# DIAGNijmegen/bodyct-dram-emph-subtype

Hardware: AMD Instinct MI355X
Metric: CT volumes/sec (train step, 1x128x256x256) (higher is better)
Workload: dtype f32; 1 GPU; BASELINE configs[1]: resnet18segcls train step (fwd+loss+bwd+Adam), batch 2/GPU, 1x128x256x256, fp32, inputs resident in HBM; global_batch=2, parallelism=dp1, hip_graph=False, streams=2

## Files before the change

### bodyct-dram-emph-subtype_amd/csrc/stem.hip

```cpp
#include "common.h"

namespace {

constexpr int PZ = 13, PY = 21, PX = 21;
constexpr int PATCH = PZ * PY * PX;
constexpr int PXP = 24;
constexpr int PATCHP = PZ * PY * PXP;
constexpr int WLP = 96;
constexpr int KT = 50;
constexpr int WPT = (KT * 64 + 255) / 256;

struct StemGeom {
  int B, D, H, W, Do, Ho, Wo;
  int nz, ny, nx, tiles_per_b, nblk;
};

template <typename T>
__global__ __launch_bounds__(256, 2) void stem_fwd_kernel(const float* __restrict__ x,
                                                          const float* __restrict__ w,
                                                          T* __restrict__ y, float* __restrict__ stats,
                                                          const StemGeom g) {
  __shared__ __attribute__((aligned(16))) float lds[PATCHP + KT * WLP];
  float* patch = lds;
  float* wl = lds + PATCHP;
  const int tid = threadIdx.x, lane = tid & 63, wave = tid >> 6;
  const int li = lane & 31, lh = lane >> 5;

  int L = xcd_remap(blockIdx.x, g.nblk);
  const int b = L / g.tiles_per_b;
  int r = L - b * g.tiles_per_b;
  const int txi = r % g.nx; r /= g.nx;
  const int tyi = r % g.ny;
  const int tzi = r / g.ny;
  const int z0 = tzi * 4, y0 = tyi * 8, x0 = txi * 8;

  for (int idx = tid; idx < PATCH; idx += 256) {
    const int pz = idx / (PY * PX);
    const int rem = idx - pz * (PY * PX);
    const int py = rem / PX, px = rem - py * PX;
    const int zi = 2 * z0 - 3 + pz, yi = 2 * y0 - 3 + py, xi = 2 * x0 - 3 + px;
    const bool ok = (zi >= 0) & (zi < g.D) & (yi >= 0) & (yi < g.H) & (xi >= 0) & (xi < g.W);
    patch[(pz * PY + py) * PXP + px] = ok ? x[(((long)b * g.D + zi) * g.H + yi) * g.W + xi] : 0.f;
  }

  float rw[WPT];
  auto load_w = [&](int kz) {
#pragma unroll
    for (int p = 0; p < WPT; ++p) {
      const int idx = p * 256 + tid;
      const int t = idx >> 6, co = idx & 63;
      rw[p] = (idx < KT * 64 && t < 49) ? w[co * 343 + kz * 49 + t] : 0.f;
    }
  };
  auto store_w = [&]() {
#pragma unroll
    for (int p = 0; p < WPT; ++p) {
      const int idx = p * 256 + tid;
      if (idx < KT * 64) wl[(idx >> 6) * WLP + (idx & 63)] = rw[p];
    }
  };

  f32x16 acc[2][2];
#pragma unroll
  for (int mi = 0; mi < 2; ++mi)
#pragma unroll
    for (int nj = 0; nj < 2; ++nj)
#pragma unroll
      for (int e = 0; e < 16; ++e) acc[mi][nj][e] = 0.f;

  int abase[2];
#pragma unroll
  for (int mi = 0; mi < 2; ++mi) abase[mi] = (2 * wave) * (PY * PXP) + (2 * (4 * mi + (li >> 3))) * PXP + 2 * (li & 7);

  load_w(0);
  for (int kz = 0; kz < 7; ++kz) {
    __syncthreads();
    store_w();
    __syncthreads();
    if (kz + 1 < 7) load_w(kz + 1);
    const float* pk = patch + kz * (PY * PXP);
#pragma unroll
    for (int kk = 0; kk < KT / 2; ++kk) {
      constexpr int dummy = 0;
      (void)dummy;
      const int k0 = 2 * kk, k1 = 2 * kk + 1;
      const int o0 = (k0 < 49) ? (k0 / 7) * PXP + (k0 % 7) : 0;
      const int o1 = (k1 < 49) ? (k1 / 7) * PXP + (k1 % 7) : 0;
      const int ko = lh ? o1 : o0;
      const float a0 = pk[abase[0] + ko];
      const float a1 = pk[abase[1] + ko];
      const float b0 = wl[(2 * kk + lh) * WLP + li];
      const float b1 = wl[(2 * kk + lh) * WLP + 32 + li];
      acc[0][0] = __builtin_amdgcn_mfma_f32_32x32x2f32(a0, b0, acc[0][0], 0, 0, 0);
      acc[0][1] = __builtin_amdgcn_mfma_f32_32x32x2f32(a0, b1, acc[0][1], 0, 0, 0);
      acc[1][0] = __builtin_amdgcn_mfma_f32_32x32x2f32(a1, b0, acc[1][0], 0, 0, 0);
      acc[1][1] = __builtin_amdgcn_mfma_f32_32x32x2f32(a1, b1, acc[1][1], 0, 0, 0);
    }
  }

  float s1[2] = {0.f, 0.f}, s2[2] = {0.f, 0.f};
#pragma unroll
  for (int mi = 0; mi < 2; ++mi) {
#pragma unroll
    for (int e = 0; e < 16; ++e) {
      const int row = wave * 64 + mi * 32 + (e & 3) + 8 * (e >> 2) + 4 * lh;
      const int zo = z0 + (row >> 6), yo = y0 + ((row >> 3) & 7), xo = x0 + (row & 7);
      if ((zo < g.Do) & (yo < g.Ho) & (xo < g.Wo)) {
        const long o = ((((long)b * g.Do + zo) * g.Ho + yo) * g.Wo + xo) * 64 + li;
#pragma unroll
        for (int nj = 0; nj < 2; ++nj) {
          const float v = acc[mi][nj][e];
          st1<T>(y, o + nj * 32, v);
          s1[nj] += v;
          s2[nj] += v * v;
        }
      }
    }
  }
  if (stats) {
    __syncthreads();
    float* red = lds;
#pragma unroll
    for (int nj = 0; nj < 2; ++nj) {
      const float t1 = s1[nj] + __shfl_xor(s1[nj], 32, 64);
      const float t2 = s2[nj] + __shfl_xor(s2[nj], 32, 64);
      if (lh == 0) {
        red[(wave * 2 + 0) * 64 + nj * 32 + li] = t1;
        red[(wave * 2 + 1) * 64 + nj * 32 + li] = t2;
      }
    }
    __syncthreads();
    if (tid < 128) {
      const int which = tid >> 6, c = tid & 63;
      const float v = red[(0 + which) * 64 + c] + red[(2 + which) * 64 + c] + red[(4 + which) * 64 + c] +
                      red[(6 + which) * 64 + c];
      stats[((long)L * 2 + which) * 64 + c] = v;
    }
  }
}

constexpr int GZ = 7, GY = 21, GX = 21;
constexpr int GPATCH = GZ * GY * GX;
constexpr int GXP = 27;
constexpr int GPATCHP = GZ * GY * GXP;
constexpr int NTAP = 352;
constexpr int GLDY = 96;
constexpr int GPT = (GPATCH + 255) / 256;

struct StemWGeom {
  int B, D, H, W, Do, Ho, Wo;
  int ny, nx;
  int total;
};

template <typename T>
__global__ __launch_bounds__(256, 2) void stem_wgrad_kernel(const float* __restrict__ x,
                                                            const T* __restrict__ dy,
                                                            float* __restrict__ slab, const StemWGeom g) {
  __shared__ __attribute__((aligned(16))) float lds[GPATCHP + 3 + 64 * GLDY];
  float* patch = lds;
  float* dyl = lds + GPATCHP + 3;
  const int tid = threadIdx.x, lane = tid & 63, wave = tid >> 6;
  const int li = lane & 31, lh = lane >> 5;
  const int ntw = (wave < 3) ? 3 : 2;

  int toff[3];
#pragma unroll
  for (int j = 0; j < 3; ++j) {
    const int tap = 32 * (wave + 4 * j) + li;
    const int kz = tap / 49, rem = tap - kz * 49, ky = rem / 7, kx = rem - ky * 7;
    toff[j] = (tap < 343 ? kz * (GY * GXP) + ky * GXP + kx : 0) + 2 * lh;
  }

  f32x16 acc[3][2];
#pragma unroll
  for (int j = 0; j < 3; ++j)
#pragma unroll
    for (int mi = 0; mi < 2; ++mi)
#pragma unroll
      for (int e = 0; e < 16; ++e) acc[j][mi][e] = 0.f;

  float rp[GPT];
  float4 rd[4];
  auto load_tile = [&](int st) {
    int r = st;
    const int txi = r % g.nx; r /= g.nx;
    const int tyi = r % g.ny; r /= g.ny;
    const int zo = r % g.Do;
    const int b = r / g.Do;
    const int y0 = tyi * 8, x0 = txi * 8;
#pragma unroll
    for (int p = 0; p < GPT; ++p) {
      const int idx = p * 256 + tid;
      const int pz = idx / (GY * GX);
      const int rem = idx - pz * (GY * GX);
      const int py = rem / GX, px = rem - py * GX;
      const int zi = 2 * zo - 3 + pz, yi = 2 * y0 - 3 + py, xi = 2 * x0 - 3 + px;
      const bool ok = (idx < GPATCH) & (zi >= 0) & (zi < g.D) & (yi >= 0) & (yi < g.H) & (xi >= 0) & (xi < g.W);
      rp[p] = ok ? x[(((long)b * g.D + zi) * g.H + yi) * g.W + xi] : 0.f;
    }
#pragma unroll
    for (int p = 0; p < 4; ++p) {
      const int idx = p * 256 + tid;
      const int v = idx >> 4, c4 = idx & 15;
      const int yo = y0 + (v >> 3), xo = x0 + (v & 7);
      const bool ok = (yo < g.Ho) & (xo < g.Wo);
      const long o = ((((long)b * g.Do + zo) * g.Ho + yo) * g.Wo + xo) * 64 + c4 * 4;
      rd[p] = ok ? ld4<T>(dy, o) : make_float4(0.f, 0.f, 0.f, 0.f);
    }
  };
  auto store_tile = [&]() {
#pragma unroll
    for (int p = 0; p < GPT; ++p) {
      const int idx = p * 256 + tid;
      if (idx < GPATCH) {
        const int pz = idx / (GY * GX), rem = idx - pz * (GY * GX);
        patch[(pz * GY + rem / GX) * GXP + rem % GX] = rp[p];
      }
    }
#pragma unroll
    for (int p = 0; p < 4; ++p) {
      const int idx = p * 256 + tid;
      *reinterpret_cast<float4*>(&dyl[(idx >> 4) * GLDY + (idx & 15) * 4]) = rd[p];
    }
  };

  int st = blockIdx.x;
  if (st < g.total) load_tile(st);
  for (; st < g.total; st += gridDim.x) {
    __syncthreads();
    store_tile();
    __syncthreads();
    if (st + (int)gridDim.x < g.total) load_tile(st + gridDim.x);
#pragma unroll 8
    for (int kk = 0; kk < 32; ++kk) {
      const int vbase = (2 * (kk >> 2)) * GXP + 4 * (kk & 3);
      const float a0 = dyl[(2 * kk + lh) * GLDY + li];
      const float a1 = dyl[(2 * kk + lh) * GLDY + 32 + li];
#pragma unroll
      for (int j = 0; j < 3; ++j) {
        if (j < ntw) {
          const float bv = patch[vbase + toff[j]];
          acc[j][0] = __builtin_amdgcn_mfma_f32_32x32x2f32(a0, bv, acc[j][0], 0, 0, 0);
          acc[j][1] = __builtin_amdgcn_mfma_f32_32x32x2f32(a1, bv, acc[j][1], 0, 0, 0);
        }
      }
    }
  }
  float* sl = slab + (long)blockIdx.x * 64 * NTAP;
#pragma unroll
  for (int j = 0; j < 3; ++j) {
    if (j < ntw) {
#pragma unroll
      for (int mi = 0; mi < 2; ++mi)
#pragma unroll
        for (int e = 0; e < 16; ++e) {
          const int co = 32 * mi + (e & 3) + 8 * (e >> 2) + 4 * lh;
          sl[co * NTAP + 32 * (wave + 4 * j) + li] = acc[j][mi][e];
        }
    }
  }
}

__global__ __launch_bounds__(256) void stem_wgrad_reduce_kernel(const float* __restrict__ slab, float* __restrict__ dw,
                                                                int nslab) {
  __shared__ float part[4][64];
  const int r = threadIdx.x & 63, kg = threadIdx.x >> 6;
  const int i = blockIdx.x * 64 + r;
  const bool live = i < 64 * NTAP;
  float p[8];
#pragma unroll
  for (int j = 0; j < 8; ++j) p[j] = 0.f;
  if (live) {
    int k = kg;
    for (; k + 28 < nslab; k += 32) {
#pragma unroll
      for (int j = 0; j < 8; ++j) p[j] += slab[(long)(k + 4 * j) * 64 * NTAP + i];
    }
    for (int j = 0; k < nslab; k += 4, ++j) p[j] += slab[(long)k * 64 * NTAP + i];
  }
  part[kg][r] = ((p[0] + p[1]) + (p[2] + p[3])) + ((p[4] + p[5]) + (p[6] + p[7]));
  __syncthreads();
  if (kg == 0 && live) {
    const int co = i / NTAP, tap = i - co * NTAP;
    if (tap < 343) dw[co * 343 + tap] = (part[0][r] + part[1][r]) + (part[2][r] + part[3][r]);
  }
}

inline int stem_out(int n) { return (n + 6 - 7) / 2 + 1; }
inline int stem_wgrad_blocks(int total) { return total < 512 ? total : 512; }

}

extern "C" int dram_stem_num_tiles(int B, int Do, int Ho, int Wo) {
  return B * ((Do + 3) / 4) * ((Ho + 7) / 8) * ((Wo + 7) / 8);
}

template <typename T>
static int stem_fwd_impl(const float* x, const float* w, T* y, float* stats_partial, int B, int D, int H, int W,
                         dram_stream_t stream) {
  if (!x || !w || !y || B < 1 || D < 1 || H < 1 || W < 1) return DRAM_ERR_BAD_ARG;
  StemGeom g{};
  g.B = B; g.D = D; g.H = H; g.W = W;
  g.Do = stem_out(D); g.Ho = stem_out(H); g.Wo = stem_out(W);
  if ((long long)B * g.Do * g.Ho * g.Wo * 64 >= (1LL << 31)) return DRAM_ERR_UNSUPPORTED;
  g.nz = (g.Do + 3) / 4; g.ny = (g.Ho + 7) / 8; g.nx = (g.Wo + 7) / 8;
  g.tiles_per_b = g.nz * g.ny * g.nx;
  g.nblk = B * g.tiles_per_b;
  const double vo = (double)B * g.Do * g.Ho * g.Wo;
  DramProf prof(DRAM_FAM_STEM, 0, 2.0 * vo * 64.0 * 343.0,
                4.0 * ((double)B * D * H * W + 64.0 * 343.0) + sizeof(T) * vo * 64.0, (hipStream_t)stream);
  hipLaunchKernelGGL((stem_fwd_kernel<T>), dim3(g.nblk), dim3(256), 0, (hipStream_t)stream, x, w, y, stats_partial, g);
  DRAM_LAUNCH_CHECK();
  return DRAM_OK;
}
extern "C" int dram_stem_fwd(const float* x, const float* w, float* y, float* stats_partial, int B, int D,
                             int H, int W, dram_stream_t stream) {
  return stem_fwd_impl<float>(x, w, y, stats_partial, B, D, H, W, stream);
}
extern "C" int dram_stem_fwd_bf16(const float* x, const float* w, void* y, float* stats_partial, int B, int D,
                                  int H, int W, dram_stream_t stream) {
  return stem_fwd_impl<bf16_t>(x, w, (bf16_t*)y, stats_partial, B, D, H, W, stream);
}

extern "C" size_t dram_stem_bwd_weight_workspace(int B, int D, int H, int W) {
  const int Do = stem_out(D), Ho = stem_out(H), Wo = stem_out(W);
  const int total = B * Do * ((Ho + 7) / 8) * ((Wo + 7) / 8);
  return (size_t)stem_wgrad_blocks(total) * 64 * NTAP * sizeof(float);
}

template <typename T>
static int stem_bwd_weight_impl(const float* x, const T* dy, float* dw, int B, int D, int H, int W, void* workspace,
                                size_t workspace_bytes, dram_stream_t stream) {
  if (!x || !dy || !dw || B < 1 || D < 1 || H < 1 || W < 1) return DRAM_ERR_BAD_ARG;
  StemWGeom g{};
  g.B = B; g.D = D; g.H = H; g.W = W;
  g.Do = stem_out(D); g.Ho = stem_out(H); g.Wo = stem_out(W);
  g.ny = (g.Ho + 7) / 8; g.nx = (g.Wo + 7) / 8;
  g.total = B * g.Do * g.ny * g.nx;
  const int nblk = stem_wgrad_blocks(g.total);
  if (!workspace || workspace_bytes < (size_t)nblk * 64 * NTAP * sizeof(float)) return DRAM_ERR_WORKSPACE;
  hipStream_t s = (hipStream_t)stream;
  const double vo = (double)B * g.Do * g.Ho * g.Wo;
  DramProf prof(DRAM_FAM_STEM, 1, 2.0 * vo * 64.0 * 343.0,
                4.0 * ((double)B * D * H * W + 64.0 * 343.0) + sizeof(T) * vo * 64.0, s);
  hipLaunchKernelGGL((stem_wgrad_kernel<T>), dim3(nblk), dim3(256), 0, s, x, dy, (float*)workspace, g);
  DRAM_LAUNCH_CHECK();
  hipLaunchKernelGGL(stem_wgrad_reduce_kernel, dim3((64 * NTAP + 63) / 64), dim3(256), 0, s,
                     (const float*)workspace, dw, nblk);
  DRAM_LAUNCH_CHECK();
  return DRAM_OK;
}
extern "C" int dram_stem_bwd_weight(const float* x, const float* dy, float* dw, int B, int D, int H, int W,
                                    void* workspace, size_t workspace_bytes, dram_stream_t stream) {
  return stem_bwd_weight_impl<float>(x, dy, dw, B, D, H, W, workspace, workspace_bytes, stream);
}
extern "C" int dram_stem_bwd_weight_bf16(const float* x, const void* dy, float* dw, int B, int D, int H, int W,
                                         void* workspace, size_t workspace_bytes, dram_stream_t stream) {
  return stem_bwd_weight_impl<bf16_t>(x, (const bf16_t*)dy, dw, B, D, H, W, workspace, workspace_bytes, stream);
}
```

### include/dram_hip.h

```cpp
#ifndef DRAM_HIP_H
#define DRAM_HIP_H

#include <stddef.h>
#include <stdint.h>

#ifdef __cplusplus
extern "C" {
#endif

typedef void* dram_stream_t;

#define DRAM_OK 0
#define DRAM_ERR_BAD_ARG (-1)
#define DRAM_ERR_UNSUPPORTED (-2)
#define DRAM_ERR_WORKSPACE (-3)

#define DRAM_ABI_VERSION 7
int dram_version(void);
const char* dram_build_info(void);
const char* dram_abi_hash(void);
unsigned long long dram_stream_capture_id(dram_stream_t stream);

enum {
  DRAM_FAM_CONV_WINO2D = 0,
  DRAM_FAM_WINO_IN,
  DRAM_FAM_WINO_GEMM_NN,
  DRAM_FAM_WINO_OUT,
  DRAM_FAM_WINO_GEMM_TN,
  DRAM_FAM_WINO_WGRAD_OUT,
  DRAM_FAM_WEIGHT_PACK,
  DRAM_FAM_WGRAD_W2D,
  DRAM_FAM_CONV_IGEMM,
  DRAM_FAM_CONV_WGRAD,
  DRAM_FAM_STEM,
  DRAM_FAM_BN,
  DRAM_FAM_POOL_UP,
  DRAM_FAM_HEAD_LOSS,
  DRAM_FAM_OPTIM,
  DRAM_FAM_PREP,
  DRAM_FAM_CONV_BF16,
  DRAM_FAM_WGRAD_BF16,
  DRAM_FAM_COUNT
};
typedef struct DramProfRecord {
  int32_t family;
  int32_t variant;
  double mfma_flops;
  double alg_flops;
  double hbm_bytes;
  float ms;
  float pad_;
} DramProfRecord;
const char* dram_profile_family_name(int family);
int dram_profile_family_is_mfma(int family);
int dram_profile_start(int max_records);
int dram_profile_stop(void);
int dram_profile_dropped(void);
int dram_profile_read(DramProfRecord* out, int max_records);

typedef struct DramConvDesc {
  int32_t B;
  int32_t D, H, W, Cin;
  int32_t Do, Ho, Wo, Cout;
  int32_t k;
  int32_t stride, pad, dil;
  int32_t flags;
} DramConvDesc;
#define DRAM_CONV_ROUNDING_TOLERANT 1
#define DRAM_CONV_BWD_OVERLAPPED 2

int dram_pack_conv_weight(const float* w, float* wf, float* wb, int Cout, int Cin, int taps,
                          dram_stream_t stream);

int dram_conv3d_fwd(const float* x, const float* wf, const float* bias, float* y,
                    float* stats_partial, const DramConvDesc* desc, dram_stream_t stream);

int dram_conv3d_bwd_data(const float* dy, const float* wb, float* dx, const float* add,
                         const float* gate, const DramConvDesc* desc, dram_stream_t stream);

size_t dram_conv3d_bwd_weight_workspace(const DramConvDesc* desc);
int dram_conv3d_bwd_weight(const float* x, const float* dy, float* dw, const DramConvDesc* desc,
                           void* workspace, size_t workspace_bytes, dram_stream_t stream);

int dram_conv_num_mtiles(const DramConvDesc* desc);

int dram_wino_applicable(const DramConvDesc* desc);
int dram_conv_wgrad_algo(const DramConvDesc* desc);
int dram_wino_num_points(const DramConvDesc* desc);
int dram_wino_num_points_bwd(const DramConvDesc* desc);
int dram_wino_pack_weight(const float* w, float* uf, float* ub, const DramConvDesc* desc, dram_stream_t stream);
size_t dram_wino_workspace(const DramConvDesc* desc, int pass);
int dram_wino_num_stat_rows(const DramConvDesc* desc);
size_t dram_wino_v_elems(const DramConvDesc* desc);
int dram_wino_conv3d_fwd(const float* x, const float* uf, const float* bias, float* y,
                         float* stats_partial, float* v_keep, const DramConvDesc* desc, void* workspace,
                         size_t workspace_bytes, dram_stream_t stream);
int dram_wino_prologue_supported(const DramConvDesc* d);
int dram_wino_conv3d_fwd_cat(const float* x0, int C0, const float* x1, int C1, const float* uf, const float* bias, float* y,
                             float* stats_partial, float* v_keep, const DramConvDesc* desc, void* workspace,
                             size_t workspace_bytes, dram_stream_t stream);
int dram_wino_conv3d_fwd_bn(const float* x_pre, const float* pscale, const float* pshift, const float* uf, const float* bias,
                            float* y, float* stats_partial, float* v_keep, const DramConvDesc* d, void* workspace,
                            size_t workspace_bytes, dram_stream_t stream);
int dram_wino_conv3d_bwd_data(const float* dy, const float* ub, float* dx, const float* add,
                              const float* gate, const DramConvDesc* desc, void* workspace,
                              size_t workspace_bytes, dram_stream_t stream);
int dram_wino_num_stat_rows_bwd(const DramConvDesc* desc);
int dram_wino_conv3d_bwd_data_bn(const float* dy, const float* ub, float* dx, const float* bn_y, const float* bn_mean,
                                 const float* bn_invstd, const float* bn_scale, const float* bn_shift,
                                 float* stats_partial, const DramConvDesc* desc, void* workspace, size_t workspace_bytes,
                                 dram_stream_t stream);
int dram_wino_conv3d_bwd_weight(const float* x, const float* v_cache, const float* dy, float* dw,
                                const DramConvDesc* desc, void* workspace, size_t workspace_bytes,
                                dram_stream_t stream);

int dram_wino2d_applicable(const DramConvDesc* desc);
int dram_wino2d_num_stat_rows(const DramConvDesc* desc);
int dram_wino2d_pack_weight(const float* w, float* uf, float* ub, int Cout, int Cin, dram_stream_t stream);
int dram_wino2d_conv3d_fwd(const float* x, const float* uf, const float* bias, float* y,
                           float* stats_partial, const DramConvDesc* desc, dram_stream_t stream);
int dram_wino2d_conv3d_bwd_data(const float* dy, const float* ub, float* dx, const float* add,
                                const float* gate, const DramConvDesc* desc, dram_stream_t stream);

int dram_wgrad_w2d_applicable(const DramConvDesc* desc);
size_t dram_wgrad_w2d_workspace(const DramConvDesc* desc);
int dram_wgrad_w2d(const float* x, const float* dy, float* dw, const DramConvDesc* desc, void* workspace,
                   size_t workspace_bytes, dram_stream_t stream);

int dram_conv1x1_applicable(const DramConvDesc* desc);
int dram_conv1x1_num_stat_rows(const DramConvDesc* desc);
int dram_conv1x1_fwd(const float* x, const float* w2d, const float* bias, float* y, float* stats_partial,
                     const DramConvDesc* desc, dram_stream_t stream);
int dram_conv1x1_bwd_data(const float* dy, const float* wt, float* dx, const float* add, const float* gate,
                          const DramConvDesc* desc, dram_stream_t stream);
size_t dram_conv1x1_bwd_weight_workspace(const DramConvDesc* desc);
int dram_conv1x1_bwd_weight(const float* x, const float* dy, float* dw, const DramConvDesc* desc, void* workspace,
                            size_t workspace_bytes, dram_stream_t stream);

int dram_conv_algo(const DramConvDesc* desc);

int dram_stem_num_tiles(int B, int Do, int Ho, int Wo);
int dram_stem_fwd(const float* x, const float* w, float* y, float* stats_partial, int B, int D, int H,
                  int W, dram_stream_t stream);
size_t dram_stem_bwd_weight_workspace(int B, int D, int H, int W);
int dram_stem_bwd_weight(const float* x, const float* dy, float* dw, int B, int D, int H, int W,
                         void* workspace, size_t workspace_bytes, dram_stream_t stream);
size_t dram_stem_bwd_data_workspace(int B, int D, int H, int W);
int dram_stem_bwd_data(const float* dy, const float* w, float* dx, int B, int D, int H, int W, void* workspace,
                       size_t workspace_bytes, dram_stream_t stream);

int dram_reduce_partials_stages(int nparts);
#define DRAM_FOLD_TICKET_DOUBLES 256
int dram_fold_partials_stages(int nparts);
int dram_fold_partials(const float* partial, double* sums, double* scratch, float* sums_f32, float* f32_row1, int nparts,
                       int R, int C, double tail, int has_tail, dram_stream_t stream);
int dram_bn_fold_finalize(const float* partial, double* sums, double* scratch, int nparts, int C, double count,
                          const float* gamma, const float* beta, float* running_mean, float* running_var, float momentum,
                          float eps, int update_running, float* mean, float* invstd, float* scale, float* shift,
                          dram_stream_t stream);
int dram_reduce_partials(const float* partial, double* sums, double* scratch, int nparts, int R, int C,
                         double tail, int has_tail, dram_stream_t stream);

int dram_bn_finalize(const double* sums, double count, const double* count_dev, const float* gamma, const float* beta,
                     float* running_mean, float* running_var, float momentum, float eps,
                     int update_running, float* mean, float* invstd, float* scale, float* shift,
                     int C, dram_stream_t stream);

int dram_bn_apply(const float* y, const float* scale, const float* shift, const float* residual,
                  int Dr, int Hr, int Wr, int Cr, int rs, float* z, int B, int D, int H, int W, int C,
                  int relu, dram_stream_t stream);

int dram_colsum_nparts(long long rows, int C);
int dram_bn_bwd_reduce(const float* dz, const float* z, const float* y, const float* mean,
                       const float* invstd, const float* scale, const float* shift, float* partial,
                       long long rows, int C, int relu, dram_stream_t stream);
int dram_bn_bwd_apply_nparts(long long rows, int C);
int dram_bn_bwd_apply(const float* dz, const float* z, const float* y, const float* mean,
                      const float* invstd, const float* gamma, const float* scale, const float* shift,
                      const double* sums, double count, const double* count_dev, float* dy,
                      float* colsum_partial, long long rows, int C, int relu, dram_stream_t stream);
int dram_bn_bwd_apply_eval(const float* dz, const float* z, const float* y, const float* scale, const float* shift,
                           float* dy, float* colsum_partial, long long rows, int C, int relu, dram_stream_t stream);
int dram_colsum(const float* a, float* partial, long long rows, int C, dram_stream_t stream);

int dram_maxpool_fwd(const float* x, float* y, uint8_t* argmax, int B, int D, int H, int W, int C,
                     dram_stream_t stream);
int dram_bn_maxpool_fwd(const float* y, const float* scale, const float* shift, float* z, float* pooled, uint8_t* argmax,
                        int B, int D, int H, int W, int C, dram_stream_t stream);
int dram_maxpool_bwd(const float* dy, const uint8_t* argmax, const float* add, int add_stride, float* dx,
                     int B, int D, int H, int W, int C, dram_stream_t stream);

int dram_upcat_fwd(const float* src, const float* skip, float* cat, int B, int Ds, int Hs, int Ws, int Cu,
                   int Dk, int Hk, int Wk, int Ck, dram_stream_t stream);
int dram_upcat_bwd(const float* dcat, float* dsrc, float* dskip, int B, int Ds, int Hs, int Ws, int Cu,
                   int Dk, int Hk, int Wk, int Ck, dram_stream_t stream);

int dram_upmix_stat_rows(long long nvox);
int dram_upmix_axis_fwd(const void* in, int in_bf16, float* out, long long outer, int Ni, int m, int C,
                        dram_stream_t stream);
int dram_upmix_axis_fwd_final(const float* in, const void* base, void* out, int out_bf16, float* stats, long long outer,
                              int Ni, int m, int C, dram_stream_t stream);
int dram_upmix_axis_bwd(const void* g, int g_bf16, void* h, int h_bf16, long long outer, int Ni, int m, int C,
                        dram_stream_t stream);
int dram_upmix_split_weight(const float* w, float* wlo, float* ws, int Co, int Cu, int Cs, dram_stream_t stream);
int dram_upmix_merge_wgrad(const float* dwlo, const float* dws, float* dw, int Co, int Cu, int Cs, dram_stream_t stream);

int dram_head_nblk(long long voxels_per_sample);
int dram_head_fwd(const float* x, const float* w, const float* bias, const float* lungs, int Dl, int Hl,
                  int Wl, float* dense, float* partial, int B, int D, int H, int W, int NO, int sigmoid,
                  dram_stream_t stream);
int dram_head_bwd_nparts(long long voxels_per_sample);
int dram_head_bwd(const float* x, const float* w, const float* dense, const float* gdense,
                  const float* gpool, const float* lungs, int Dl, int Hl, int Wl, float* dx,
                  float* wpartial, int B, int D, int H, int W, int NO, int sigmoid, dram_stream_t stream);

#define DRAM_CAM_GRADCAM 0
#define DRAM_CAM_HIRESCAM 1
#define DRAM_CAM_LAYERCAM 2
int dram_cam_nblk(long long voxels_per_sample);
int dram_cam_point(const float* x, const float* w, const float* bias, const float* gdense, const float* gpool,
                   const float* lungs, int Dl, int Hl, int Wl, float* out, int B, int D, int H, int W, int NO,
                   int sigmoid, int method, int relu, dram_stream_t stream);
int dram_cam_sum(const float* x, const float* w, const float* bias, const float* gdense, const float* gpool,
                 const float* lungs, int Dl, int Hl, int Wl, float* partial, int B, int D, int H, int W, int NO,
                 int sigmoid, dram_stream_t stream);
int dram_cam_combine(const float* x, const float* w, const double* sums, float* out, int B, int D, int H, int W,
                     int NO, int relu, dram_stream_t stream);

int dram_segloss_nblk(long long voxels_total);
int dram_segloss_fwd(const float* cle, const float* pse, const float* lungs, const float* ems,
                     const float* binary, int Dl, int Hl, int Wl, float* partial, int B, int D, int H,
                     int W, float smoothness, dram_stream_t stream);
int dram_segloss_bwd(const float* cle, const float* pse, const float* lungs, const float* ems,
                     const float* binary, int Dl, int Hl, int Wl, const float* coef, float* gcle,
                     float* gpse, int B, int D, int H, int W, float smoothness, dram_stream_t stream);

int dram_regloss_tail(const float* partial, int nblk, const float* reg_cle, const float* reg_pse,
                      const long long* cle_labels, const long long* pse_labels, const float* cle_w,
                      const float* pse_w, const float* cle_bands, int n_cle, const float* pse_bands, int n_pse,
                      int B, double voxels_total, double smooth, double beta, double gamma, float* out,
                      float* coef, float* greg, dram_stream_t stream);

int dram_upproject_nblk(long long voxels_per_sample);
int dram_upproject(const float* dense, const float* ess, float* out, float* partial, int B, int D, int H,
                   int W, int Do, int Ho, int Wo, dram_stream_t stream);

int dram_region_nblk(long long voxels_per_sample);
int dram_upproject_regions(const float* cle, const float* pse, long long dense_batch_stride, const uint8_t* ess,
                           const uint8_t* labels, float* out_cle, float* out_pse, float* partial, double* table, int B,
                           int D, int H, int W, int Do, int Ho, int Wo, int n_regions, dram_stream_t stream);
int dram_prep_labels(const void* labels, int label_dtype, long long stride_z, long long stride_y, const int* zidx,
                     uint8_t* out, int D, int H, int W, int Do, int Ho, int Wo, dram_stream_t stream);

#define DRAM_HEAT_CLASSSUM 0
#define DRAM_HEAT_PLAIN 1
int dram_heat_nblk(long long voxels_per_sample);
int dram_heat_peak(const float* dense, long long stride_b, long long stride_c, int C, float* partial, int B, int d,
                   int h, int w, int D, int H, int W, dram_stream_t stream);
int dram_heat_volume(const float* dense, long long stride_b, long long stride_c, int C, const uint8_t* lung,
                     const float* peak, const int* zsel, int nz, float* out_f32, uint8_t* out_u8, int mode, int B,
                     int d, int h, int w, int D, int H, int W, dram_stream_t stream);

typedef struct DramTensorRef {
  float* p;
  const float* g;
  float* m;
  float* v;
  int64_t n;
} DramTensorRef;
typedef struct DramChunkRef {
  int32_t tensor;
  int32_t pad;
  int64_t offset;
} DramChunkRef;
#define DRAM_OPT_CHUNK 16384
typedef struct DramPackRef {
  const float* w;
  int64_t off_f;
  int64_t off_b;
  int32_t Cout, Cin, taps, pad;
} DramPackRef;
int dram_adam_multi(const DramTensorRef* table, const DramChunkRef* chunks, int nchunks, float lr,
                    float beta1, float beta2, float eps, float weight_decay, float bias_corr1,
                    float bias_corr2, float grad_scale, dram_stream_t stream);
int dram_adam_multi_dev(const DramTensorRef* table, const DramChunkRef* chunks, int nchunks, float* hyper,
                        dram_stream_t stream);
int dram_sgd_multi(const DramTensorRef* table, const DramChunkRef* chunks, int nchunks, float lr,
                   float momentum, float weight_decay, int first_step, float grad_scale,
                   dram_stream_t stream);

int dram_grad_norm_multi(const DramTensorRef* table, const DramChunkRef* chunks, int nchunks, double* partials,
                         float* clip, float grad_scale, const float* hyper, dram_stream_t stream);
int dram_grad_scale_multi(const DramTensorRef* table, const DramChunkRef* chunks, int nchunks, const float* clip,
                          dram_stream_t stream);
int dram_adam_multi_clip(const DramTensorRef* table, const DramChunkRef* chunks, int nchunks, float lr,
                         float beta1, float beta2, float eps, float weight_decay, float bias_corr1,
                         float bias_corr2, float grad_scale, const float* clip, dram_stream_t stream);
int dram_adam_multi_dev_clip(const DramTensorRef* table, const DramChunkRef* chunks, int nchunks, float* hyper,
                             const float* clip, dram_stream_t stream);
int dram_sgd_multi_clip(const DramTensorRef* table, const DramChunkRef* chunks, int nchunks, float lr,
                        float momentum, float weight_decay, int first_step, float grad_scale, const float* clip,
                        dram_stream_t stream);

int dram_window_stats_nblk(long long n);
int dram_window_stats(const float* scan, float* partial, long long n, float lo, float hi, dram_stream_t stream);
int dram_prep_image(const float* scan, const int* zidx, const float* mean_invstd, float* out, int D, int H, int W,
                    int Do, int Ho, int Wo, float lo, float hi, dram_stream_t stream);
int dram_prep_mask(const float* mask, const int* zidx, float* out, int D, int H, int W, int Do, int Ho, int Wo,
                   dram_stream_t stream);

int dram_sample_stats_nblk(long long n);
int dram_sample_stats_i16(const int16_t* scan, long long* partial, long long n, int lo, int hi, dram_stream_t stream);
int dram_prep_sample_i16(const int16_t* scan, const void* lung, int lung_dtype, const int* zidx, const float* mean_invstd,
                         float* out_image, uint8_t* out_lung, uint8_t* out_em, int D, int H, int W, int Do, int Ho, int Wo,
                         int lo, int hi, int em_threshold, dram_stream_t stream);

int dram_resample_paste(const float* src, float* out_f32, uint8_t* out_u8, int D, int H, int W, int rd, int rh, int rw,
                        int oz, int oy, int ox, int Do, int Ho, int Wo, dram_stream_t stream);

int dram_lung_bbox_nblk(long long n);
int dram_lung_bbox(const void* lobes, int lobe_dtype, int* partial, int* box, int D, int H, int W,
                   dram_stream_t stream);
int dram_case_prepare(const void* scan, const void* lobes, int lobe_dtype, void* image, uint8_t* lung_mask,
                      uint8_t* ess_mask, void* original, int D, int H, int W, int z0, int y0, int x0, int Dc, int Hc,
                      int Wc, int radius, int fill_value, int threshold, dram_stream_t stream);

int dram_lobe_hist_nblk(long long voxels);
int dram_lobe_hist(const void* image, const void* labels, int label_dtype, long long stride_z, long long stride_y,
                   int* part_hist, int64_t* part_sums, int64_t* hist, int64_t* sums, int D, int H, int W, int n_regions,
                   int hu_lo, int nbins, dram_stream_t stream);

long long dram_lung_zones_workspace(int D, int H, int W, long long max_um);
int dram_lung_zones(const void* labels, int label_dtype, long long stride_z, long long stride_y, uint8_t* zones,
                    uint8_t* zone_labels, float* dist_mm, void* workspace, int D, int H, int W, int sz_um, int sy_um,
                    int sx_um, long long peel_um, long long max_um, int n_regions, dram_stream_t stream);

long long dram_lobe_zones_workspace(int D, int H, int W, long long max_um);
int dram_lobe_zones(const void* labels, int label_dtype, long long stride_z, long long stride_y, uint8_t* zones,
                    uint8_t* zone_labels, float* pleura_mm, float* fissure_mm_out, void* workspace, int D, int H, int W,
                    int sz_um, int sy_um, int sx_um, long long peel_um, long long fissure_um, long long max_um,
                    int n_regions, dram_stream_t stream);

size_t dram_label_components_workspace(int D, int H, int W);
int dram_label_components(const void* key_or_labels, int lab_elem, long long stride_z, long long stride_y,
                          const int16_t* image, int threshold, int by_lobe, int connectivity, int n_regions,
                          int32_t* components, int32_t* cluster_voxels, int64_t* table, void* work, int D, int H, int W,
                          dram_stream_t stream);

long long dram_component_shapes_workspace(int D, int H, int W);
int dram_component_rank(const int32_t* components, void* work, int64_t* count, int D, int H, int W,
                        dram_stream_t stream);
int dram_component_shapes(const int32_t* components, const void* labels, int lab_elem, long long stride_z,
                          long long stride_y, const uint8_t* zones, const void* work, int64_t* rows, long long capacity,
                          int64_t* count, int D, int H, int W, dram_stream_t stream);

int dram_median3d(const int16_t* in, int16_t* out, int D, int H, int W, int rz, int ry, int rx, dram_stream_t stream);

#define DRAM_GAUSS_NEAREST 0
#define DRAM_GAUSS_ZERO 1
typedef struct DramGaussTaps {
  int32_t radius[3];
  float w[3][17];
} DramGaussTaps;
long long dram_gauss3d_workspace(int D, int z0, int Do, int Ho, int Wo, int rz);
int dram_gauss3d(const void* in, int in_type, void* out, int out_type, int D, int H, int W, int z0, int y0, int x0,
                 int Do, int Ho, int Wo, const DramGaussTaps* taps, int border, void* work, long long work_bytes,
                 dram_stream_t stream);

typedef struct DramAugment {
  int32_t flags;
  int32_t n_boxes;
  int32_t boxes[10][6];
  int32_t flip_axes;
  float sigma;
  float box_lo[3];
  float box_hi[3];
} DramAugment;
int dram_minmax_nblk(long long n);
int dram_minmax(const float* x, float* partial, long long n, dram_stream_t stream);
int dram_augment_image(const float* x, const float* noise, const float* minmax, float* out, int D, int H, int W,
                       const DramAugment* aug, dram_stream_t stream);
int dram_augment_mask(const float* mask, float* out, int D, int H, int W, const DramAugment* aug,
                      dram_stream_t stream);

int dram_add(const float* a, const float* b, float* out, long long n, dram_stream_t stream);

long long dram_pack_conv_weight_bf16_tiles(int Cout, int Cin, int taps);
int dram_pack_conv_weight_bf16_multi(const DramPackRef* table, const DramChunkRef* chunks, int nchunks, void* flat,
                                     double total_elems, dram_stream_t stream);
int dram_cast_f32_to_bf16(const float* src, void* dst, long long n, dram_stream_t stream);
int dram_cast_bf16_to_f32(const void* src, float* dst, long long n, dram_stream_t stream);
int dram_s2d_bf16(const void* x, void* x8, int B, int D, int H, int W, int C, dram_stream_t stream);
int dram_d2s_bf16(const void* dx8, const void* add, const void* gate, void* dx, int B, int D, int H, int W, int C,
                  dram_stream_t stream);
int dram_s2_embed_weight(const float* w, float* w3, int Cout, int Cin, dram_stream_t stream);
int dram_s2_extract_wgrad(const float* dw3, float* dw, int Cout, int Cin, dram_stream_t stream);
int dram_conv_bf16_supported(const DramConvDesc* d);
int dram_conv_bf16_num_stat_rows(const DramConvDesc* d);
int dram_pack_conv_weight_bf16(const float* w, void* wf, void* wb, int Cout, int Cin, int taps, dram_stream_t stream);
int dram_conv3d_fwd_bf16(const void* x, const void* wf, const float* bias, void* y, float* stats_partial,
                         const DramConvDesc* d, dram_stream_t stream);
int dram_conv3d_bwd_data_bf16(const void* dy, const void* wb, void* dx, const void* add, const void* gate,
                              const DramConvDesc* d, dram_stream_t stream);
size_t dram_conv3d_bwd_weight_bf16_workspace(const DramConvDesc* d);
int dram_conv3d_bwd_weight_bf16(const void* x, const void* dy, float* dw, const DramConvDesc* d, void* workspace,
                                size_t workspace_bytes, dram_stream_t stream);
int dram_stem_fwd_bf16(const float* x, const float* w, void* y, float* stats_partial, int B, int D, int H, int W,
                       dram_stream_t stream);
int dram_stem_bwd_weight_bf16(const float* x, const void* dy, float* dw, int B, int D, int H, int W, void* workspace,
                              size_t workspace_bytes, dram_stream_t stream);
int dram_stem_bwd_data_bf16(const void* dy, const float* w, float* dx, int B, int D, int H, int W, void* workspace,
                            size_t workspace_bytes, dram_stream_t stream);
int dram_stem_fwd_bf16mm(const float* x, const float* w, void* y, float* stats_partial, int B, int D, int H, int W,
                         dram_stream_t stream);
int dram_stem_bwd_weight_bf16mm(const float* x, const void* dy, float* dw, int B, int D, int H, int W, void* workspace,
                                size_t workspace_bytes, dram_stream_t stream);
int dram_stem_fwd_blocks(int ntile);
int dram_bn_apply_bf16(const void* y, const float* scale, const float* shift, const void* residual, int Dr, int Hr,
                       int Wr, int Cr, int rs, void* z, int B, int D, int H, int W, int C, int relu,
                       dram_stream_t stream);
int dram_bn_bwd_reduce_bf16(const void* dz, const void* z, const void* y, const float* mean, const float* invstd,
                            const float* scale, const float* shift, float* partial, long long rows, int C, int relu,
                            dram_stream_t stream);
int dram_bn_bwd_apply_bf16(const void* dz, const void* z, const void* y, const float* mean, const float* invstd,
                           const float* gamma, const float* scale, const float* shift, const double* sums, double count,
                           const double* count_dev, void* dy, float* colsum_partial, long long rows, int C, int relu,
                           dram_stream_t stream);
int dram_bn_bwd_apply_eval_bf16(const void* dz, const void* z, const void* y, const float* scale, const float* shift,
                                void* dy, float* colsum_partial, long long rows, int C, int relu, dram_stream_t stream);
int dram_colsum_bf16(const void* a, float* partial, long long rows, int C, dram_stream_t stream);
int dram_maxpool_fwd_bf16(const void* x, void* y, uint8_t* argmax, int B, int D, int H, int W, int C,
                          dram_stream_t stream);
int dram_bn_maxpool_fwd_bf16(const void* y, const float* scale, const float* shift, void* z, void* pooled, uint8_t* argmax,
                             int B, int D, int H, int W, int C, dram_stream_t stream);
int dram_maxpool_bwd_bf16(const void* dy, const uint8_t* argmax, const void* add, int add_stride, void* dx, int B, int D,
                          int H, int W, int C, dram_stream_t stream);
int dram_upcat_fwd_bf16(const void* src, const void* skip, void* cat, int B, int Ds, int Hs, int Ws, int Cu, int Dk,
                        int Hk, int Wk, int Ck, dram_stream_t stream);
int dram_upcat_bwd_bf16(const void* dcat, void* dsrc, void* dskip, int B, int Ds, int Hs, int Ws, int Cu, int Dk, int Hk,
                        int Wk, int Ck, dram_stream_t stream);
int dram_head_fwd_bf16(const void* x, const float* w, const float* bias, const float* lungs, int Dl, int Hl, int Wl,
                       float* dense, float* partial, int B, int D, int H, int W, int NO, int sigmoid,
                       dram_stream_t stream);
int dram_head_bwd_bf16(const void* x, const float* w, const float* dense, const float* gdense, const float* gpool,
                       const float* lungs, int Dl, int Hl, int Wl, void* dx, float* wpartial, int B, int D, int H, int W,
                       int NO, int sigmoid, dram_stream_t stream);
int dram_cam_point_bf16(const void* x, const float* w, const float* bias, const float* gdense, const float* gpool,
                        const float* lungs, int Dl, int Hl, int Wl, float* out, int B, int D, int H, int W, int NO,
                        int sigmoid, int method, int relu, dram_stream_t stream);
int dram_cam_sum_bf16(const void* x, const float* w, const float* bias, const float* gdense, const float* gpool,
                      const float* lungs, int Dl, int Hl, int Wl, float* partial, int B, int D, int H, int W, int NO,
                      int sigmoid, dram_stream_t stream);
int dram_cam_combine_bf16(const void* x, const float* w, const double* sums, float* out, int B, int D, int H, int W,
                          int NO, int relu, dram_stream_t stream);

#ifdef __cplusplus
}
#endif
#endif
```

Measured before the change: 55.41 volumes/sec.

## Add persistent weight-resident stem forward kernel and pipeline stem wgrad MFMA loop

Adds a persistent 512-thread stem forward kernel. Each half-block processes a tile while the full 7x7x7 weight image stays resident in LDS, which removes per-tile weight reloads. Patch loads for the next tile are prefetched into registers, and operands are software-pipelined around MFMA with sched barriers. The weight-gradient kernel gets precomputed packed offsets and a register-prefetched MFMA loop specialized per tap count. The cost is large LDS use (limiting occupancy to one block per CU), more register pressure, and a heuristic selector.

```diff
diff --git a/bodyct-dram-emph-subtype_amd/csrc/stem.hip b/bodyct-dram-emph-subtype_amd/csrc/stem.hip
--- a/bodyct-dram-emph-subtype_amd/csrc/stem.hip
+++ b/bodyct-dram-emph-subtype_amd/csrc/stem.hip
@@ -1,3 +1,4 @@
+#include <type_traits>
 #include "common.h"
 
 namespace {
@@ -139,6 +140,207 @@
   }
 }
 
+constexpr int WRP = 64;
+constexpr int WPLANE = KT * WRP;
+constexpr int WIMG = 7 * WPLANE;
+constexpr int RPT = (PATCH + 255) / 256;
+constexpr int TURN = 1632;
+constexpr int TPITCH = 64;
+constexpr int RES_LDS = 2 * PATCHP + 2 * 512 + WIMG;
+constexpr int RES_MAX_BLOCKS = 256;
+static_assert(4 * TURN <= PATCHP && 16 * TPITCH <= TURN && TURN % 4 == 0 && PATCHP % 4 == 0 && WIMG % 4 == 0, "turn");
+static_assert(RES_LDS * 4 <= 160 * 1024, "LDS");
+
+template <typename T>
+__global__ __launch_bounds__(512) void stem_fwd_res_kernel(const float* __restrict__ x, const float* __restrict__ w,
+                                                           T* __restrict__ y, float* __restrict__ stats,
+                                                           const StemGeom g, const int trips) {
+  __shared__ __attribute__((aligned(16))) float lds[RES_LDS];
+  float* wimg = lds + 2 * PATCHP + 2 * 512;
+  const int tid = threadIdx.x, lane = tid & 63;
+  const int half = __builtin_amdgcn_readfirstlane(tid >> 8);
+  const int ht = tid & 255;
+  const int wave = __builtin_amdgcn_readfirstlane(ht >> 6);
+  const int li = lane & 31, lh = lane >> 5;
+  float* patch = lds + half * PATCHP;
+  float* red = lds + 2 * PATCHP + half * 512;
+
+  for (int it = tid >> 6; it < 8 * 43; it += 8) {
+    const int co = 8 * (it & 7) + (lane >> 3), tap = 8 * (it >> 3) + (lane & 7);
+    if (tap < 343) {
+      const int kz = tap / 49;
+      wimg[(kz * KT + tap - kz * 49) * WRP + co] = w[co * 343 + tap];
+    }
+  }
+  if (tid < 7 * 64) wimg[((tid >> 6) * KT + 49) * WRP + (tid & 63)] = 0.f;
+
+  int pk[RPT];
+#pragma unroll
+  for (int p = 0; p < RPT; ++p) {
+    const int idx = p * 256 + ht;
+    const int pz = idx / (PY * PX);
+    const int rem = idx - pz * (PY * PX);
+    const int py = rem / PX, px = rem - py * PX;
+    pk[p] = idx < PATCH ? (((pz * PY + py) * PXP + px) | (pz << 13) | (py << 17) | (px << 22)) : -1;
+  }
+  float rp[RPT];
+  auto load_patch = [&](int t) __attribute__((always_inline)) {
+    const int b = t / g.tiles_per_b;
+    int r = t - b * g.tiles_per_b;
+    const int txi = r % g.nx; r /= g.nx;
+    const int tyi = r % g.ny;
+    const int tzi = r / g.ny;
+    const int zb = 8 * tzi - 3, yb = 16 * tyi - 3, xb = 16 * txi - 3;
+    unsigned uh = g.H, uw = g.W;
+    asm volatile("" : "+s"(uh), "+s"(uw));
+    const float* xt = x + ((((long)b * g.D + zb) * g.H + yb) * g.W + xb);
+#pragma unroll
+    for (int p = 0; p < RPT; ++p) {
+      int k = pk[p];
+      asm volatile("" : "+v"(k));
+      const int pz = (k >> 13) & 15, py = (k >> 17) & 31, px = (k >> 22) & 31;
+      const bool ok = (k >= 0) & ((unsigned)(zb + pz) < (unsigned)g.D) & ((unsigned)(yb + py) < (unsigned)g.H) &
+                      ((unsigned)(xb + px) < (unsigned)g.W);
+      rp[p] = ok ? xt[((unsigned)pz * uh + (unsigned)py) * uw + (unsigned)px] : 0.f;
+    }
+  };
+  auto store_patch = [&]() __attribute__((always_inline)) {
+#pragma unroll
+    for (int p = 0; p < RPT; ++p)
+      if (p < RPT - 1 || pk[p] >= 0) patch[pk[p] & 8191] = rp[p];
+  };
+
+  int abase[2];
+#pragma unroll
+  for (int mi = 0; mi < 2; ++mi) abase[mi] = (2 * wave) * (PY * PXP) + (2 * (4 * mi + (li >> 3))) * PXP + 2 * (li & 7);
+  const float* pa[2][3];
+#pragma unroll
+  for (int mi = 0; mi < 2; ++mi) {
+    pa[mi][0] = patch + abase[mi] + lh;
+    pa[mi][1] = patch + abase[mi] + lh * (PXP - 6);
+    pa[mi][2] = patch + abase[mi] - lh * (6 * PXP + 6);
+  }
+  float* turn = patch + wave * TURN;
+  const int rrow = lane >> 4, rc4 = lane & 15;
+
+  int t = 2 * blockIdx.x + half;
+  const int tstep = 2 * gridDim.x;
+  if (t < g.nblk) load_patch(t);
+  for (int trip = 0; trip < trips; ++trip, t += tstep) {
+    const bool live = t < g.nblk;
+    if (live) store_patch();
+    __syncthreads();
+    if (t + tstep < g.nblk) load_patch(t + tstep);
+
+    f32x16 acc[2][2];
+#pragma unroll
+    for (int mi = 0; mi < 2; ++mi)
+#pragma unroll
+      for (int nj = 0; nj < 2; ++nj)
+#pragma unroll
+        for (int e = 0; e < 16; ++e) acc[mi][nj][e] = 0.f;
+    if (live) {
+      const float* wl0 = wimg + lh * WRP + li;
+      float a0 = pa[0][0][0], a1 = pa[1][0][0], b0 = wl0[0], b1 = wl0[32];
+#pragma unroll 1
+      for (int kz = 0; kz < 7; ++kz) {
+        const int kzo = kz * (PY * PXP);
+        const float* wl = wl0 + kz * WPLANE;
+#pragma unroll
+        for (int kk = 0; kk < KT / 2; ++kk) {
+          const float c0 = a0, c1 = a1, d0 = b0, d1 = b1;
+          if (kk + 1 < KT / 2) {
+            const int k0 = 2 * (kk + 1);
+            const int o0 = (k0 / 7) * PXP + (k0 % 7);
+            const int cls = (k0 == 48) ? 2 : (k0 % 7 == 6) ? 1 : 0;
+            a0 = pa[0][cls][kzo + o0];
+            a1 = pa[1][cls][kzo + o0];
+            b0 = wl[k0 * WRP];
+            b1 = wl[k0 * WRP + 32];
+          } else if (kz + 1 < 7) {
+            a0 = pa[0][0][kzo + PY * PXP];
+            a1 = pa[1][0][kzo + PY * PXP];
+            b0 = wl[WPLANE];
+            b1 = wl[WPLANE + 32];
+          }
+          __builtin_amdgcn_sched_barrier(0);
+          acc[0][0] = __builtin_amdgcn_mfma_f32_32x32x2f32(c0, d0, acc[0][0], 0, 0, 0);
+          acc[0][1] = __builtin_amdgcn_mfma_f32_32x32x2f32(c0, d1, acc[0][1], 0, 0, 0);
+          acc[1][0] = __builtin_amdgcn_mfma_f32_32x32x2f32(c1, d0, acc[1][0], 0, 0, 0);
+          acc[1][1] = __builtin_amdgcn_mfma_f32_32x32x2f32(c1, d1, acc[1][1], 0, 0, 0);
+          __builtin_amdgcn_sched_barrier(0);
+        }
+      }
+    }
+    __syncthreads();
+    if (live) {
+      const int b = t / g.tiles_per_b;
+      int r = t - b * g.tiles_per_b;
+      const int txi = r % g.nx; r /= g.nx;
+      const int tyi = r % g.ny;
+      const int tzi = r / g.ny;
+      const int zo = tzi * 4 + wave, y0 = tyi * 8, x0 = txi * 8;
+      if (stats) {
+        float s1[2] = {0.f, 0.f}, s2[2] = {0.f, 0.f};
+#pragma unroll
+        for (int mi = 0; mi < 2; ++mi) {
+#pragma unroll
+          for (int e = 0; e < 16; ++e) {
+            const int row = mi * 32 + (e & 3) + 8 * (e >> 2) + 4 * lh;
+            const int yo = y0 + (row >> 3), xo = x0 + (row & 7);
+            if ((zo < g.Do) & (yo < g.Ho) & (xo < g.Wo)) {
+#pragma unroll
+              for (int nj = 0; nj < 2; ++nj) {
+                const float v = acc[mi][nj][e];
+                s1[nj] += v;
+                s2[nj] += v * v;
+              }
+            }
+          }
+        }
+#pragma unroll
+        for (int nj = 0; nj < 2; ++nj) {
+          const float t1 = s1[nj] + __shfl_xor(s1[nj], 32, 64);
+          const float t2 = s2[nj] + __shfl_xor(s2[nj], 32, 64);
+          if (lh == 0) {
+            red[(wave * 2 + 0) * 64 + nj * 32 + li] = t1;
+            red[(wave * 2 + 1) * 64 + nj * 32 + li] = t2;
+          }
+        }
+      }
+#pragma unroll
+      for (int mi = 0; mi < 2; ++mi) {
+#pragma unroll
+        for (int eh = 0; eh < 2; ++eh) {
+          __builtin_amdgcn_wave_barrier();
+#pragma unroll
+          for (int e = 8 * eh; e < 8 * eh + 8; ++e) {
+            const int rl = (e & 3) + 8 * ((e >> 2) & 1) + 4 * lh;
+            turn[rl * TPITCH + li] = acc[mi][0][e];
+            turn[rl * TPITCH + 32 + li] = acc[mi][1][e];
+          }
+          __builtin_amdgcn_wave_barrier();
+#pragma unroll
+          for (int q = 0; q < 4; ++q) {
+            const int row = 4 * q + rrow;
+            const float4 v = *reinterpret_cast<const float4*>(turn + row * TPITCH + 4 * rc4);
+            const int yo = y0 + 4 * mi + 2 * eh + (row >> 3), xo = x0 + (row & 7);
+            if ((zo < g.Do) & (yo < g.Ho) & (xo < g.Wo))
+              st4<T>(y, ((((long)b * g.Do + zo) * g.Ho + yo) * g.Wo + xo) * 64 + 4 * rc4, v);
+          }
+        }
+      }
+    }
+    __syncthreads();
+    if (live && stats && ht < 128) {
+      const int which = ht >> 6, c = ht & 63;
+      const float v = red[(0 + which) * 64 + c] + red[(2 + which) * 64 + c] + red[(4 + which) * 64 + c] +
+                      red[(6 + which) * 64 + c];
+      stats[((long)t * 2 + which) * 64 + c] = v;
+    }
+  }
+}
+
 constexpr int GZ = 7, GY = 21, GX = 21;
 constexpr int GPATCH = GZ * GY * GX;
 constexpr int GXP = 27;
@@ -160,7 +362,8 @@
   __shared__ __attribute__((aligned(16))) float lds[GPATCHP + 3 + 64 * GLDY];
   float* patch = lds;
   float* dyl = lds + GPATCHP + 3;
-  const int tid = threadIdx.x, lane = tid & 63, wave = tid >> 6;
+  const int tid = threadIdx.x, lane = tid & 63;
+  const int wave = __builtin_amdgcn_readfirstlane(tid >> 6);
   const int li = lane & 31, lh = lane >> 5;
   const int ntw = (wave < 3) ? 3 : 2;
 
@@ -180,6 +383,21 @@
 #pragma unroll
       for (int e = 0; e < 16; ++e) acc[j][mi][e] = 0.f;
 
+  int pk[GPT];
+#pragma unroll
+  for (int p = 0; p < GPT; ++p) {
+    const int idx = p * 256 + tid;
+    const int pz = idx / (GY * GX);
+    const int rem = idx - pz * (GY * GX);
+    const int py = rem / GX, px = rem - py * GX;
+    pk[p] = idx < GPATCH ? (((pz * GY + py) * GXP + px) | (pz << 12) | (py << 15) | (px << 20)) : -1;
+  }
+  unsigned doff[4];
+#pragma unroll
+  for (int p = 0; p < 4; ++p) {
+    const int idx = p * 256 + tid;
+    doff[p] = (unsigned)(((idx >> 7) * g.Wo + ((idx >> 4) & 7)) * 64 + (idx & 15) * 4);
+  }
   float rp[GPT];
   float4 rd[4];
   auto load_tile = [&](int st) {
@@ -189,35 +407,33 @@
     const int zo = r % g.Do;
     const int b = r / g.Do;
     const int y0 = tyi * 8, x0 = txi * 8;
+    const int zb = 2 * zo - 3, yb = 2 * y0 - 3, xb = 2 * x0 - 3;
+    unsigned uh = g.H, uw = g.W;
+    asm volatile("" : "+s"(uh), "+s"(uw));
+    const float* xt = x + ((((long)b * g.D + zb) * g.H + yb) * g.W + xb);
 #pragma unroll
     for (int p = 0; p < GPT; ++p) {
-      const int idx = p * 256 + tid;
-      const int pz = idx / (GY * GX);
-      const int rem = idx - pz * (GY * GX);
-      const int py = rem / GX, px = rem - py * GX;
-      const int zi = 2 * zo - 3 + pz, yi = 2 * y0 - 3 + py, xi = 2 * x0 - 3 + px;
-      const bool ok = (idx < GPATCH) & (zi >= 0) & (zi < g.D) & (yi >= 0) & (yi < g.H) & (xi >= 0) & (xi < g.W);
-      rp[p] = ok ? x[(((long)b * g.D + zi) * g.H + yi) * g.W + xi] : 0.f;
-    }
+      int k = pk[p];
+      asm volatile("" : "+v"(k));
+      const int pz = (k >> 12) & 7, py = (k >> 15) & 31, px = (k >> 20) & 31;
+      const bool ok = (k >= 0) & ((unsigned)(zb + pz) < (unsigned)g.D) & ((unsigned)(yb + py) < (unsigned)g.H) &
+                      ((unsigned)(xb + px) < (unsigned)g.W);
+      rp[p] = ok ? xt[((unsigned)pz * uh + (unsigned)py) * uw + (unsigned)px] : 0.f;
+    }
+    const T* dt = dy + ((((long)b * g.Do + zo) * g.Ho + y0) * g.Wo + x0) * 64;
 #pragma unroll
     for (int p = 0; p < 4; ++p) {
-      const int idx = p * 256 + tid;
-      const int v = idx >> 4, c4 = idx & 15;
-      const int yo = y0 + (v >> 3), xo = x0 + (v & 7);
-      const bool ok = (yo < g.Ho) & (xo < g.Wo);
-      const long o = ((((long)b * g.Do + zo) * g.Ho + yo) * g.Wo + xo) * 64 + c4 * 4;
-      rd[p] = ok ? ld4<T>(dy, o) : make_float4(0.f, 0.f, 0.f, 0.f);
+      const int v = (p * 256 + tid) >> 4;
+      const bool ok = (y0 + (v >> 3) < g.Ho) & (x0 + (v & 7) < g.Wo);
+      unsigned d = doff[p];
+      asm volatile("" : "+v"(d));
+      rd[p] = ok ? ld4<T>(dt, d) : make_float4(0.f, 0.f, 0.f, 0.f);
     }
   };
   auto store_tile = [&]() {
 #pragma unroll
-    for (int p = 0; p < GPT; ++p) {
-      const int idx = p * 256 + tid;
-      if (idx < GPATCH) {
-        const int pz = idx / (GY * GX), rem = idx - pz * (GY * GX);
-        patch[(pz * GY + rem / GX) * GXP + rem % GX] = rp[p];
-      }
-    }
+    for (int p = 0; p < GPT; ++p)
+      if (p < GPT - 1 || pk[p] >= 0) patch[pk[p] & 4095] = rp[p];
 #pragma unroll
     for (int p = 0; p < 4; ++p) {
       const int idx = p * 256 + tid;
@@ -232,20 +448,41 @@
     store_tile();
     __syncthreads();
     if (st + (int)gridDim.x < g.total) load_tile(st + gridDim.x);
-#pragma unroll 8
-    for (int kk = 0; kk < 32; ++kk) {
-      const int vbase = (2 * (kk >> 2)) * GXP + 4 * (kk & 3);
-      const float a0 = dyl[(2 * kk + lh) * GLDY + li];
-      const float a1 = dyl[(2 * kk + lh) * GLDY + 32 + li];
-#pragma unroll
-      for (int j = 0; j < 3; ++j) {
-        if (j < ntw) {
-          const float bv = patch[vbase + toff[j]];
-          acc[j][0] = __builtin_amdgcn_mfma_f32_32x32x2f32(a0, bv, acc[j][0], 0, 0, 0);
-          acc[j][1] = __builtin_amdgcn_mfma_f32_32x32x2f32(a1, bv, acc[j][1], 0, 0, 0);
+    auto sweep = [&](auto ntw_c) __attribute__((always_inline)) {
+      constexpr int NTW = decltype(ntw_c)::value;
+      const float* pd = dyl + lh * GLDY + li;
+      float a0 = pd[0], a1 = pd[32], bv[3];
+#pragma unroll
+      for (int j = 0; j < 3; ++j) bv[j] = patch[toff[j]];
+#pragma unroll 1
+      for (int ko = 0; ko < 4; ++ko) {
+        const float* pdk = pd + ko * (16 * GLDY);
+        const float* pk0 = patch + ko * (4 * GXP);
+#pragma unroll
+        for (int ki = 0; ki < 8; ++ki) {
+          const float c0 = a0, c1 = a1, cb[3] = {bv[0], bv[1], bv[2]};
+          if (ki + 1 < 8 || ko + 1 < 4) {
+            const int kn = ki + 1, vbase = (2 * (kn >> 2)) * GXP + 4 * (kn & 3);
+            a0 = pdk[2 * kn * GLDY];
+            a1 = pdk[2 * kn * GLDY + 32];
+#pragma unroll
+            for (int j = 0; j < 3; ++j)
+              if (j < NTW) bv[j] = pk0[vbase + toff[j]];
+          }
+          __builtin_amdgcn_sched_barrier(0);
+#pragma unroll
+          for (int j = 0; j < 3; ++j) {
+            if (j < NTW) {
+              acc[j][0] = __builtin_amdgcn_mfma_f32_32x32x2f32(c0, cb[j], acc[j][0], 0, 0, 0);
+              acc[j][1] = __builtin_amdgcn_mfma_f32_32x32x2f32(c1, cb[j], acc[j][1], 0, 0, 0);
+            }
+          }
+          __builtin_amdgcn_sched_barrier(0);
         }
       }
-    }
+    };
+    if (ntw == 3) sweep(std::integral_constant<int, 3>{});
+    else sweep(std::integral_constant<int, 2>{});
   }
   float* sl = slab + (long)blockIdx.x * 64 * NTAP;
 #pragma unroll
@@ -296,10 +533,20 @@
   return B * ((Do + 3) / 4) * ((Ho + 7) / 8) * ((Wo + 7) / 8);
 }
 
+constexpr int RES_MIN_TILES_PER_HALF = 1;
+static bool stem_res_fits(int H, int W) { return 13LL * H * W < (1LL << 31); }
+static int stem_fwd_form_of(long long ntile, int H, int W) {
+  return (stem_res_fits(H, W) && ntile > (long long)RES_MIN_TILES_PER_HALF * 2 * RES_MAX_BLOCKS) ? 1 : 0;
+}
+extern "C" int dram_stem_fwd_form_of(int B, int D, int H, int W) {
+  if (B < 1 || D < 1 || H < 1 || W < 1) return DRAM_ERR_BAD_ARG;
+  return stem_fwd_form_of((long long)B * ((stem_out(D) + 3) / 4) * ((stem_out(H) + 7) / 8) * ((stem_out(W) + 7) / 8), H, W);
+}
+
 template <typename T>
 static int stem_fwd_impl(const float* x, const float* w, T* y, float* stats_partial, int B, int D, int H, int W,
-                         dram_stream_t stream) {
-  if (!x || !w || !y || B < 1 || D < 1 || H < 1 || W < 1) return DRAM_ERR_BAD_ARG;
+                         dram_stream_t stream, int form = -1, int max_blocks = 0) {
+  if (!x || !w || !y || B < 1 || D < 1 || H < 1 || W < 1 || form > 1 || max_blocks < 0) return DRAM_ERR_BAD_ARG;
   StemGeom g{};
   g.B = B; g.D = D; g.H = H; g.W = W;
   g.Do = stem_out(D); g.Ho = stem_out(H); g.Wo = stem_out(W);
@@ -307,12 +554,29 @@
   g.nz = (g.Do + 3) / 4; g.ny = (g.Ho + 7) / 8; g.nx = (g.Wo + 7) / 8;
   g.tiles_per_b = g.nz * g.ny * g.nx;
   g.nblk = B * g.tiles_per_b;
+  if (form < 0) form = stem_fwd_form_of(g.nblk, H, W);
+  if (form == 1 && !stem_res_fits(H, W)) return DRAM_ERR_UNSUPPORTED;
   const double vo = (double)B * g.Do * g.Ho * g.Wo;
   DramProf prof(DRAM_FAM_STEM, 0, 2.0 * vo * 64.0 * 343.0,
                 4.0 * ((double)B * D * H * W + 64.0 * 343.0) + sizeof(T) * vo * 64.0, (hipStream_t)stream);
-  hipLaunchKernelGGL((stem_fwd_kernel<T>), dim3(g.nblk), dim3(256), 0, (hipStream_t)stream, x, w, y, stats_partial, g);
+  if (form == 1) {
+    int grid = (g.nblk + 1) / 2;
+    if (grid > RES_MAX_BLOCKS) grid = RES_MAX_BLOCKS;
+    if (max_blocks > 0 && grid > max_blocks) grid = max_blocks;
+    const int trips = (g.nblk + 2 * grid - 1) / (2 * grid);
+    hipLaunchKernelGGL((stem_fwd_res_kernel<T>), dim3(grid), dim3(512), 0, (hipStream_t)stream, x, w, y, stats_partial,
+                       g, trips);
+  } else {
+    hipLaunchKernelGGL((stem_fwd_kernel<T>), dim3(g.nblk), dim3(256), 0, (hipStream_t)stream, x, w, y, stats_partial, g);
+  }
   DRAM_LAUNCH_CHECK();
   return DRAM_OK;
+}
+extern "C" int dram_stem_fwd_form(const float* x, const float* w, void* y, float* stats_partial, int B, int D, int H,
+                                  int W, int storage, int form, int max_blocks, dram_stream_t stream) {
+  if (form < 0 || (storage != 0 && storage != 1)) return DRAM_ERR_BAD_ARG;
+  return storage ? stem_fwd_impl<bf16_t>(x, w, (bf16_t*)y, stats_partial, B, D, H, W, stream, form, max_blocks)
+                 : stem_fwd_impl<float>(x, w, (float*)y, stats_partial, B, D, H, W, stream, form, max_blocks);
 }
 extern "C" int dram_stem_fwd(const float* x, const float* w, float* y, float* stats_partial, int B, int D,
                              int H, int W, dram_stream_t stream) {
diff --git a/include/dram_hip.h b/include/dram_hip.h
--- a/include/dram_hip.h
+++ b/include/dram_hip.h
@@ -142,6 +142,9 @@
 int dram_stem_num_tiles(int B, int Do, int Ho, int Wo);
 int dram_stem_fwd(const float* x, const float* w, float* y, float* stats_partial, int B, int D, int H,
                   int W, dram_stream_t stream);
+int dram_stem_fwd_form_of(int B, int D, int H, int W);
+int dram_stem_fwd_form(const float* x, const float* w, void* y, float* stats_partial, int B, int D, int H, int W,
+                       int storage, int form, int max_blocks, dram_stream_t stream);
 size_t dram_stem_bwd_weight_workspace(int B, int D, int H, int W);
 int dram_stem_bwd_weight(const float* x, const float* dy, float* dw, int B, int D, int H, int W,
                          void* workspace, size_t workspace_bytes, dram_stream_t stream);
```

After: 55.59 volumes/sec, median of 2. About the same (+0.3%).
